# erkinov-wtf/dct

Hardware: AMD Instinct MI355X
Metric: 8x8 macroblocks/sec (DCT+quant); % HBM roofline (higher is better)
Workload: dtype fp32

## Files before the change

### dct_amd/__init__.py

```python
from __future__ import annotations

import ctypes as C
import os

HERE = os.path.dirname(os.path.abspath(__file__))
LIB_PATH = os.path.join(HERE, "libdct_amd.so")

KINDS = {"uniform": 0, "smooth": 1, "const": 2, "extreme": 3}


class DctqError(RuntimeError):
    pass


class _Plane(C.Structure):
    _fields_ = [("pixels", C.c_void_p), ("stride", C.c_longlong), ("frame_stride", C.c_longlong),
                ("width", C.c_int), ("height", C.c_int), ("nframes", C.c_int)]


_lib = None
_diag = None
DIAG_PATH = os.path.join(HERE, "libdct_amd_diag.so")


def _bind(L: C.CDLL, diagnostic: bool) -> C.CDLL:
    vp, i, ll = C.c_void_p, C.c_int, C.c_longlong
    sig = {
        "dctq_plan_create": ([i, i, C.POINTER(vp)], i),
        "dctq_plan_destroy": ([vp], None),
        "dctq_plan_set_fallback_counter": ([vp, vp], i),
        "dctq_forward_quant": ([vp, C.POINTER(_Plane), vp, vp, vp], i),
        "dctq_forward_quant_planes": ([vp, C.POINTER(_Plane), i, vp, vp, vp], i),
        "dctq_round_trip_planes": ([vp, C.POINTER(_Plane), i, vp, vp, vp, vp], i),
        "dctq_encode_workspace_bytes": ([ll], C.c_size_t),
        "dctq_encode_planes": ([vp, C.POINTER(_Plane), i, vp, vp, vp, ll, vp, vp], i),
        "dctq_encode_planes16": ([vp, C.POINTER(_Plane), i, vp, vp, vp, ll, vp, vp], i),
        "dctq_abi_version": ([], i),
        "dctq_forward_float": ([vp, C.POINTER(_Plane), vp, vp], i),
        "dctq_inverse": ([vp, vp, vp, ll, vp, vp], i),
        "dctq_decode_planes": ([vp, vp, vp, C.POINTER(_Plane), i, vp], i),
        "dctq_synth": ([C.c_uint64, i, C.POINTER(_Plane), vp], i),
        "dctq_error_string": ([i], C.c_char_p),
        "dctq_synchronize": ([vp], i),
        "dctq_rle_workspace_bytes": ([ll], C.c_size_t),
        "dctq_rle_count": ([vp, ll, vp, vp, vp], i),
        "dctq_rle_emit": ([vp, ll, vp, vp, vp], i),
        "dctq_rle_decode": ([vp, vp, ll, vp, vp], i),
        "dctq_rle_decode16": ([vp, vp, ll, vp, vp], i),
        "dctq_plan_symbol_bytes": ([vp], i),
        "dctq_huffman_bits": ([vp, ll, vp, vp], i),
        "dctq_huffman_bits_planes": ([vp, C.POINTER(_Plane), i, vp, vp], i),
        "dctq_stream_release": ([vp], i),
    }
    if diagnostic:
        sig.update({
            "dctq_diag_plan_set_variant": ([vp, i], i),
            "dctq_diag_forward_quant_planes": ([vp, C.POINTER(_Plane), i, vp, vp, vp], i),
            "dctq_diag_forward_float": ([vp, C.POINTER(_Plane), vp, vp], i),
            "dctq_diag_inverse": ([vp, vp, vp, ll, vp, vp], i),
            "dctq_diag_plan_set_num_cus": ([vp, i], i),
            "dctq_diag_plan_set_inverse": ([vp, i], i),
            "dctq_debug_inverse_bound": ([i, i, C.POINTER(i)], C.c_double),
            "dctq_debug_symbol_bytes": ([i, i], i),
            "dctq_diag_legacy_lanes": ([C.POINTER(i), C.POINTER(i)], i),
            "dctq_diag_movement_planes": ([vp, C.POINTER(_Plane), i, vp, vp], i),
            "dctq_diag_movement_v2_planes": ([vp, C.POINTER(_Plane), i, vp, vp], i),
            "dctq_diag_movement_grid_planes": ([vp, C.POINTER(_Plane), i, vp, i, vp], i),
            "dctq_diag_rt_movement_planes": ([vp, C.POINTER(_Plane), i, vp, vp, vp], i),
            "dctq_diag_stream": ([i, vp, vp, ll, vp], i),
            "dctq_diag_stream_release": ([vp], i),
            "dctq_debug_tables": ([i, i, vp, vp, vp, vp], i),
            "dctq_debug_fastdiv": ([C.c_uint32, C.c_uint32], i),
            "dctq_debug_dc_table": ([i, vp], i),
            "dctq_debug_forward_kernel": ([i, i, ll, i], i),
            "dctq_diag_stream_stash_bytes": ([vp], ll),
        })
    for name, (args, res) in sig.items():
        fn = getattr(L, name)
        fn.argtypes = args
        fn.restype = res
    return L


def lib() -> C.CDLL:
    global _lib
    if _lib is None:
        if not os.path.exists(LIB_PATH):
            raise DctqError(f"{LIB_PATH} is missing: run `python -m dct_amd.build` (hipcc, gfx950)")
        _lib = _bind(C.CDLL(LIB_PATH), False)
    return _lib


def diag() -> C.CDLL:
    global _diag
    if _diag is None:
        if not os.path.exists(DIAG_PATH):
            raise DctqError(f"{DIAG_PATH} is missing: run `python -m dct_amd.build` (hipcc, gfx950)")
        _diag = _bind(C.CDLL(DIAG_PATH), True)
    return _diag


def _check(rc: int, L: C.CDLL = None) -> None:
    if rc != 0:
        raise DctqError(f"dctq error {rc}: {(L or lib()).dctq_error_string(rc).decode()}")


def _need(t, numel: int, dtype, what: str, device=None):
    import torch
    if not isinstance(t, torch.Tensor) or not t.is_cuda:
        raise DctqError(f"{what} must be a tensor on a HIP device")
    if t.dtype != dtype:
        raise DctqError(f"{what} must be {dtype}, got {t.dtype}")
    if not t.is_contiguous():
        raise DctqError(f"{what} must be contiguous")
    if t.numel() < numel:
        raise DctqError(f"{what} holds {t.numel()} elements, {numel} needed")
    if device is not None and t.device != device:
        raise DctqError(f"{what} is on {t.device}, the input is on {device}")
    return t


def _stream_ptr(stream=None):
# ... 329 lines not shown
```

### dct_amd/build.py

```python
from __future__ import annotations

import os
import re
import subprocess
import sys

HERE = os.path.dirname(os.path.abspath(__file__))
ROOT = os.path.dirname(HERE)
CSRC = os.path.join(HERE, "csrc")
LIB = os.path.join(HERE, "libdct_amd.so")
DIAG_LIB = os.path.join(HERE, "libdct_amd_diag.so")
DIAG_SOURCES = ["diag.hip", "fdct8_diag.hip"]
SOURCES = ["api.hip", "legacy.hip", "fdct8.hip", "fdct8_aux.hip", "f64_pair.hip", "rle.hip", "roundtrip.hip", "encode.hip", "huffman.hip", "decode.hip"]
HEADERS = ["dctq_internal.h", "plan.h", "dctq_diag.h", "fdct8_bound.h", "idct8_bound.h", "host_tables.h", "aan_f64.h", "fdct8_core.h", "pair_core.h", "inverse_core.h", "scan_core.h", "zigzag.h"]
ARCH = "gfx950"


INFO = os.path.join(HERE, "build_info.json")


def _sha256(path: str) -> str:
    import hashlib
    with open(path, "rb") as f:
        return hashlib.sha256(f.read()).hexdigest()


def _inputs() -> dict:
    deps = [os.path.join(CSRC, f) for f in SOURCES + DIAG_SOURCES + HEADERS] + [os.path.abspath(__file__)]
    deps += [os.path.join(ROOT, "include", f) for f in sorted(os.listdir(os.path.join(ROOT, "include")))]
    return {os.path.relpath(d, ROOT): _sha256(d) for d in deps}


def build_info() -> dict:
    import json
    try:
        with open(INFO) as f:
            return json.load(f)
    except (OSError, ValueError):
        return {}


def _stale() -> bool:
    if not os.path.exists(LIB) or not os.path.exists(DIAG_LIB):
        return True
    info = build_info()
    return (info.get("inputs") != _inputs() or info.get("lib_sha256") != _sha256(LIB)
            or info.get("diag_sha256") != _sha256(DIAG_LIB) or info.get("flags") != _portable_flags())


def _portable_flags() -> list:
    return [f.replace(ROOT, "$ROOT") for f in _flags()]


def _flags():
    return ["hipcc", f"--offload-arch={ARCH}", "-O3", "-std=c++17", "-fPIC", "-ffp-contract=off",
            "-fno-slp-vectorize", "-Wall", "-Wno-unused-command-line-argument",
            "-I" + os.path.join(ROOT, "include"), "-I" + CSRC]


def declared_functions(headers) -> list:
    names = set()
    for h in headers:
        src = re.sub(r"/\*.*?\*/", "", open(h).read(), flags=re.S)
        for m in re.finditer(r"^[A-Za-z_][\w \*]*?\b([a-z_][a-z0-9_]*)\s*\(", src, flags=re.M):
            if m.group(1) not in ("if", "while", "for", "return", "sizeof", "defined"):
                names.add(m.group(1))
    return sorted(names)
# ... 60 lines not shown
```

### dct_amd/csrc/api.hip

```cpp
#include <dlfcn.h>
#include <math.h>
#include <stdio.h>
#include <stdlib.h>
#include <string.h>

#include <atomic>
#include <functional>
#include <map>
#include <mutex>
#include <string>
#include <thread>
#include <utility>
#include <vector>

#include "dct_amd.h"
#include "dctq_diag.h"
#include "dctq_internal.h"
#include "fdct8_bound.h"
#include "host_tables.h"
#include "idct8_bound.h"
#include "plan.h"

namespace {
thread_local std::string g_err;
// ... 419 lines not shown
                               symbols ? (unsigned long long)symbols_capacity : 0ull, workspace, (hipStream_t)stream,
                               plan->num_cus),
           "encode launch");
    return DCTQ_OK;
}

int dctq_encode_planes(const dctq_plan *plan, const dctq_plane *planes, int nplanes, int16_t *const *coef,
                       uint32_t *offsets, uint32_t *symbols, long long symbols_capacity, void *workspace,
                       void *stream) {
    DCTQ_LAUNCH(stream, 2);
    return encode_planes(plan, planes, nplanes, coef, offsets, symbols, symbols_capacity, workspace, stream, 4);
}

int dctq_encode_planes16(const dctq_plan *plan, const dctq_plane *planes, int nplanes, int16_t *const *coef,
                         uint32_t *offsets, uint16_t *symbols, long long symbols_capacity, void *workspace,
                         void *stream) {
    DCTQ_LAUNCH(stream, 13);
    return encode_planes(plan, planes, nplanes, coef, offsets, symbols, symbols_capacity, workspace, stream, 2);
}

int dctq_forward_quant(const dctq_plan *plan, const dctq_plane *src, int16_t *coef, int32_t *var_num, void *stream) {
    if (!src) return fail(DCTQ_EINVAL, "plane is NULL");
    return dctq_forward_quant_planes(plan, src, 1, &coef, var_num ? &var_num : nullptr, stream);
}

int dctq_forward_float(const dctq_plan *plan, const dctq_plane *src, float *coef, void *stream) {
    DCTQ_LAUNCH(stream, 3);
    if (int rc = dctq::check_plan(plan)) return rc;
    if (!coef) return fail(DCTQ_EINVAL, "coef is NULL");
    if (((uintptr_t)coef) % 16) return fail(DCTQ_EINVAL, "coef must be 16-byte aligned");
    dctq::PlaneArgs a;
    int rc = dctq::plane_args(src, &a);
    if (rc) return rc;
    HIPCHK(dctq::launch_fdct8_float_pair(a, plan->dev, coef, (hipStream_t)stream, plan->num_cus),
           "fdct8_float_pair launch");
    return DCTQ_OK;
}

int dctq_inverse(const dctq_plan *plan, const int16_t *coef, const int32_t *var_num, long long nblocks, float *recon,
                 void *stream) {
    DCTQ_LAUNCH(stream, 4);
    if (int rc = dctq::check_plan(plan)) return rc;
    if (!coef || !recon) return fail(DCTQ_EINVAL, "coef/recon is NULL");
    if (plan->adaptive && !var_num) return fail(DCTQ_EINVAL, "adaptive inverse needs var_num");
    if (nblocks < 0 || nblocks >= (1ll << 40)) return fail(DCTQ_EINVAL, "bad nblocks");
    if (((uintptr_t)coef) % 16 || ((uintptr_t)recon) % 16) return fail(DCTQ_EINVAL, "coef/recon must be 16-byte aligned");
    if (nblocks == 0) return DCTQ_OK;
    HIPCHK(dctq::launch_idct8_pair(plan->dev, plan->adaptive, coef, var_num, nblocks, recon, (hipStream_t)stream,
                                   plan->num_cus),
           "idct8_pair launch");
    return DCTQ_OK;
}

int dctq_decode_planes(const dctq_plan *plan, const int16_t *const *coef, const int32_t *const *var_num,
                       const dctq_plane *dst, int nplanes, void *stream) {
    DCTQ_LAUNCH(stream, 14);
    if (int rc = dctq::check_plan(plan)) return rc;
    if (!coef || !dst) return fail(DCTQ_EINVAL, "coef/dst is NULL");
    if (nplanes < 1 || nplanes > dctq::kMaxPlanes) return fail(DCTQ_EINVAL, "nplanes must be in [1, 4]");
    if (plan->adaptive && !var_num) return fail(DCTQ_EINVAL, "adaptive decode needs var_num");
    dctq::DecodeSet ds = {};
    ds.n = nplanes;
    uint32_t first = 0;
    for (int k = 0; k < nplanes; ++k) {
        if (int rc = dctq::plane_args(&dst[k], &ds.pl[k])) return rc;
        if (!coef[k]) return fail(DCTQ_EINVAL, "coef[k] is NULL");
        if (((uintptr_t)coef[k]) % 16) return fail(DCTQ_EINVAL, "coef must be 16-byte aligned");
        if (plan->adaptive && !var_num[k]) return fail(DCTQ_EINVAL, "adaptive decode needs every var_num[k]");
        ds.coef[k] = coef[k];
        ds.var[k] = plan->adaptive ? var_num[k] : nullptr;
        ds.first[k] = first;
        first += (uint32_t)((ds.pl[k].nblk + 31) / 32);
    }
    for (int k = nplanes; k <= dctq::kMaxPlanes; ++k) ds.first[k] = first;
    HIPCHK(dctq::launch_decode(ds, plan->dev, plan->adaptive, plan->inv_f32 != 0, (hipStream_t)stream, plan->num_cus),
           "decode launch");
    return DCTQ_OK;
}

int dctq_synth(uint64_t seed, int kind, const dctq_plane *dst, void *stream) {
    DCTQ_LAUNCH(stream, 5);
    if (!dst || !dst->pixels) return fail(DCTQ_EINVAL, "dst is NULL");
    if (dst->width <= 0 || dst->height <= 0 || dst->width % 4 || dst->stride < dst->width || dst->stride % 4 ||
        dst->nframes < 1 || ((uintptr_t)dst->pixels) % 4)
        return fail(DCTQ_EINVAL, "bad synth plane geometry");
    HIPCHK(dctq::launch_synth(seed, kind, (uint8_t *)dst->pixels, dst->stride, dst->frame_stride, dst->width,
                              dst->height, dst->nframes, (hipStream_t)stream),
           "synth launch");
    return DCTQ_OK;
}

static int device_cus() {
    int dev = 0, n = 0;
    if (hipGetDevice(&dev) != hipSuccess) return 256;
    if (hipDeviceGetAttribute(&n, hipDeviceAttributeMultiprocessorCount, dev) != hipSuccess || n < 1) return 256;
    return n;
}

static int rle_args(const void *a, const void *b, long long nblocks) {
    if (!a || !b) return fail(DCTQ_EINVAL, "NULL pointer");
    if (nblocks < 1 || nblocks >= (1ll << 26)) return fail(DCTQ_EINVAL, "nblocks must be in [1, 2^26)");
    return DCTQ_OK;
}

size_t dctq_rle_workspace_bytes(long long nblocks) { return dctq::rle_workspace_bytes(nblocks < 1 ? 1 : nblocks); }

int dctq_rle_count(const int16_t *coef, long long nblocks, uint32_t *offsets, void *workspace, void *stream) {
    DCTQ_LAUNCH(stream, 6);
    if (int rc = rle_args(coef, offsets, nblocks)) return rc;
    if (!workspace) return fail(DCTQ_EINVAL, "workspace is NULL");
    HIPCHK(dctq::launch_rle_count(coef, nblocks, offsets, workspace, (hipStream_t)stream, device_cus()),
           "rle_count launch");
    return DCTQ_OK;
}

int dctq_rle_emit(const int16_t *coef, long long nblocks, const uint32_t *offsets, uint32_t *symbols, void *stream) {
    DCTQ_LAUNCH(stream, 7);
    if (int rc = rle_args(coef, offsets, nblocks)) return rc;
    if (!symbols) return fail(DCTQ_EINVAL, "symbols is NULL");
    HIPCHK(dctq::launch_rle_emit(coef, nblocks, offsets, symbols, 4, ~0ull, (hipStream_t)stream, device_cus()),
           "rle_emit launch");
    return DCTQ_OK;
}

int dctq_rle_decode(const uint32_t *symbols, const uint32_t *offsets, long long nblocks, int16_t *coef,
                    void *stream) {
    DCTQ_LAUNCH(stream, 8);
// ... 98 lines not shown
```

### dct_amd/csrc/dctq_diag.h

```cpp
#ifndef DCTQ_DIAG_H
#define DCTQ_DIAG_H

#include "dct_amd.h"

#ifdef __cplusplus
extern "C" {
#endif

int dctq_diag_plan_set_variant(dctq_plan *plan, int variant);
int dctq_diag_forward_quant_planes(const dctq_plan *plan, const dctq_plane *planes, int nplanes, int16_t *const *coef,
                                   int32_t *const *var_num, void *stream);
int dctq_diag_forward_float(const dctq_plan *plan, const dctq_plane *src, float *coef, void *stream);
int dctq_diag_inverse(const dctq_plan *plan, const int16_t *coef, const int32_t *var_num, long long nblocks,
                      float *recon, void *stream);

int dctq_diag_plan_set_inverse(dctq_plan *plan, int mode);

int dctq_diag_plan_set_num_cus(dctq_plan *plan, int num_cus);

int dctq_diag_movement_planes(const dctq_plan *plan, const dctq_plane *planes, int nplanes, int16_t *const *coef,
                              void *stream);
int dctq_diag_movement_grid_planes(const dctq_plan *plan, const dctq_plane *planes, int nplanes, int16_t *const *coef,
                                   int grid_mult, void *stream);
int dctq_diag_movement_v2_planes(const dctq_plan *plan, const dctq_plane *planes, int nplanes, int16_t *const *coef,
                                 void *stream);

int dctq_diag_rt_movement_planes(const dctq_plan *plan, const dctq_plane *planes, int nplanes, int16_t *const *coef,
                                 float *const *recon, void *stream);

int dctq_diag_stream(int kind, const void *src, void *dst, long long blocks, void *stream);

int dctq_diag_stream_release(void *stream);
long long dctq_diag_stream_stash_bytes(void *stream);

int dctq_debug_forward_kernel(int quality, int adaptive, long long batches, int num_cus);
int dctq_debug_tables(int quality, int adaptive, float *w, float *thr, double *dct, double *quant);
int dctq_debug_dc_table(int quality, int16_t *out);
int dctq_debug_fastdiv(uint32_t d, uint32_t n);
double dctq_debug_inverse_bound(int quality, int adaptive, int *admitted);
int dctq_debug_symbol_bytes(int quality, int adaptive);
int dctq_diag_legacy_lanes(int *made, int *pooled);

#ifdef __cplusplus
}
#endif
#endif
```

### dct_amd/csrc/decode.hip

```cpp
#include "inverse_core.h"

namespace dctq {

constexpr int kDecodeGridMult = 64;

__device__ __forceinline__ const int16_t *coef_in(const DecodeSet &ds, int k) {
    const int16_t *c = ds.coef[0];
#pragma unroll
    for (int i = 1; i < kMaxPlanes; ++i) c = k == i ? ds.coef[i] : c;
    return c;
}
__device__ __forceinline__ const int32_t *var_in(const DecodeSet &ds, int k) {
    const int32_t *v = ds.var[0];
#pragma unroll
    for (int i = 1; i < kMaxPlanes; ++i) v = k == i ? ds.var[i] : v;
    return v;
}
__device__ __forceinline__ uint32_t first_batch(const DecodeSet &ds, int k) {
    uint32_t f = 0u;
#pragma unroll
    for (int i = 1; i < kMaxPlanes; ++i) f = k == i ? ds.first[i] : f;
    return f;
}
__device__ __forceinline__ int plane_of_batch(const DecodeSet &ds, uint32_t g) {
    int k = 0;
#pragma unroll
    for (int i = 1; i < kMaxPlanes; ++i) k += (i < ds.n && g >= ds.first[i]) ? 1 : 0;
    return k;
}

template <bool ADAPTIVE>
__device__ __forceinline__ void prefetch_coefs(const DecodeSet &ds, uint32_t g, int h, int j, uint4 (&rows)[4],
                                               int32_t &vn) {
    const int k = plane_of_batch(ds, g);
    const uint32_t n = (g - first_batch(ds, k)) * 32u + (uint32_t)j;
    const uint32_t m = n < (uint32_t)ds.pl[k].nblk ? n : 0u;
    const u4p *src = reinterpret_cast<const u4p *>(coef_in(ds, k) + (size_t)m * 64) + 4 * h;
#pragma unroll
    for (int r = 0; r < 4; ++r) {
        const u4p t = __builtin_nontemporal_load(src + r);
        rows[r] = make_uint4(t.x, t.y, t.z, t.w);
    }
    if (ADAPTIVE) vn = __builtin_nontemporal_load(var_in(ds, k) + m);
}

__device__ __forceinline__ uint32_t pack_u8x4(float a, float b, float c, float d) {
    uint32_t w = 0u;
    w = __builtin_amdgcn_cvt_pk_u8_f32(__builtin_rintf(__builtin_amdgcn_fmed3f(a, 0.0f, 255.0f)), 0u, w);
    w = __builtin_amdgcn_cvt_pk_u8_f32(__builtin_rintf(__builtin_amdgcn_fmed3f(b, 0.0f, 255.0f)), 1u, w);
    w = __builtin_amdgcn_cvt_pk_u8_f32(__builtin_rintf(__builtin_amdgcn_fmed3f(c, 0.0f, 255.0f)), 2u, w);
    w = __builtin_amdgcn_cvt_pk_u8_f32(__builtin_rintf(__builtin_amdgcn_fmed3f(d, 0.0f, 255.0f)), 3u, w);
    return w;
}

template <bool ADAPTIVE, bool INV32>
__global__ __launch_bounds__(kThreadsP, 4) void decode8(DecodeSet ds, const DevTables *__restrict__ dev) {
    const int lane = threadIdx.x & 63, wv = __builtin_amdgcn_readfirstlane(threadIdx.x >> 6);
    const int h = lane >> 5, j = lane & 31;
    const uint32_t nbatch = ds.first[kMaxPlanes];
    const uint32_t step = gridDim.x * kWavesP;
    uint32_t g = blockIdx.x * kWavesP + wv;
    uint4 nxt[4];
    int32_t nvn = 0;
    prefetch_coefs<ADAPTIVE>(ds, g, h, j, nxt, nvn);
    for (; g < nbatch; g += step) {
        const int k = plane_of_batch(ds, g);
        const PlaneArgs &p = ds.pl[k];
        const uint32_t n = (g - first_batch(ds, k)) * 32u + (uint32_t)j;
        const bool valid = n < (uint32_t)p.nblk;
        uint4 cur[4];
#pragma unroll
        for (int r = 0; r < 4; ++r) cur[r] = nxt[r];
        const int32_t vn = nvn;
        prefetch_coefs<ADAPTIVE>(ds, g + step, h, j, nxt, nvn);

        u2p pix[4];
        const auto pack = [&pix](int r, int c, const float (&o)[4]) { pix[r][c >> 2] = pack_u8x4(o[0], o[1], o[2], o[3]); };
        if constexpr (INV32) inverse_half_f32_rows(dev, cur, h, pack);
        else inverse_half_rows<ADAPTIVE>(dev, cur, vn, h, pack);

        const uint32_t m = valid ? n : 0u;
        const uint32_t f = fdiv(m, p.div_frame);
        const uint32_t rem = m - f * (uint32_t)p.nblk_frame;
        const uint32_t by = fdiv(rem, p.div_bw);
        const uint32_t bx = rem - by * (uint32_t)p.bw;
        uint8_t *base = const_cast<uint8_t *>(p.src);
        if (p.span) {
            const __amdgpu_buffer_rsrc_t rs = __builtin_amdgcn_make_buffer_rsrc(base, (short)0, (int)p.span, 0x00020000);
            const uint32_t st = (uint32_t)p.stride;
            const uint32_t off = f * (uint32_t)p.frame_stride + (by * 8u + 4u * (uint32_t)h) * st + bx * 8u;
            if (valid) {
#pragma unroll
                for (int r = 0; r < 4; ++r) __builtin_amdgcn_raw_buffer_store_b64(pix[r], rs, off + r * st, 0, kNtAux);
            }
        } else if (valid) {
            uint8_t *px = base + (long long)f * p.frame_stride + (long long)(by * 8u + 4u * (uint32_t)h) * p.stride +
                          (long long)bx * 8;
#pragma unroll
            for (int r = 0; r < 4; ++r) __builtin_nontemporal_store(pix[r], reinterpret_cast<u2p *>(px + r * p.stride));
        }
    }
}

template <bool A, bool F32>
static hipError_t launch_dec(const DecodeSet &ds, const DevTables *dev, hipStream_t stream, int num_cus) {
    static const int per_cu = resident_per_cu(decode8<A, F32>, kThreadsP);
    const uint32_t nbatch = ds.first[kMaxPlanes];
    const uint32_t want = (nbatch + kWavesP - 1) / kWavesP;
    const uint32_t cap = (uint32_t)(num_cus * per_cu * kDecodeGridMult);
    hipLaunchKernelGGL((decode8<A, F32>), dim3(want < cap ? want : cap), dim3(kThreadsP), 0, stream, ds, dev);
    return hipGetLastError();
}

hipError_t launch_decode(const DecodeSet &ds, const DevTables *dev, int adaptive, bool inv_f32, hipStream_t stream,
                         int num_cus) {
    if (adaptive) return launch_dec<true, false>(ds, dev, stream, num_cus);
    if (inv_f32) return launch_dec<false, true>(ds, dev, stream, num_cus);
    return launch_dec<false, false>(ds, dev, stream, num_cus);
}

}
```

### dct_amd/csrc/diag.hip

```cpp
#include <string.h>

#include "dctq_diag.h"
#include "fdct8_bound.h"
#include "host_tables.h"
#include "plan.h"

namespace dctq {
namespace {

typedef unsigned int u4v __attribute__((ext_vector_type(4)));
typedef unsigned int u2v2 __attribute__((ext_vector_type(2)));

template <int AUX>
__global__ __launch_bounds__(256) void stream12(const u4v *__restrict__ src, char *__restrict__ dst, uint32_t nb) {
    const int lane = threadIdx.x & 63;
    for (uint32_t b = blockIdx.x * 4 + (threadIdx.x >> 6); b < nb; b += gridDim.x * 4) {
        u4v v[4];
#pragma unroll
        for (int k = 0; k < 4; ++k) v[k] = __builtin_nontemporal_load(src + (size_t)b * 256 + k * 64 + lane);
        const __amdgpu_buffer_rsrc_t rc = __builtin_amdgcn_make_buffer_rsrc(dst + (size_t)b * 8192, 0, 8192, 0x00020000);
#pragma unroll
        for (int k = 0; k < 4; ++k) {
            __builtin_amdgcn_raw_buffer_store_b128(v[k], rc, lane * 16, k * 1024, AUX);
            __builtin_amdgcn_raw_buffer_store_b128(v[k] ^ u4v{1, 0, 0, 0}, rc, lane * 16, (k + 4) * 1024, AUX);
        }
    }
}

__global__ __launch_bounds__(256) void stream124(const u4v *__restrict__ src, char *__restrict__ dst, uint32_t nb) {
    const int lane = threadIdx.x & 63;
    for (uint32_t b = blockIdx.x * 4 + (threadIdx.x >> 6); b < nb; b += gridDim.x * 4) {
        u4v v[4];
#pragma unroll
        for (int k = 0; k < 4; ++k) v[k] = __builtin_nontemporal_load(src + (size_t)b * 256 + k * 64 + lane);
        const __amdgpu_buffer_rsrc_t rc =
            __builtin_amdgcn_make_buffer_rsrc(dst + (size_t)b * 24576, 0, 24576, 0x00020000);
#pragma unroll
        for (int k = 0; k < 4; ++k)
#pragma unroll
            for (int m = 0; m < 6; ++m)
                __builtin_amdgcn_raw_buffer_store_b128(v[k] ^ u4v{(unsigned)m, 0, 0, 0}, rc, lane * 16,
                                                       (k * 6 + m) * 1024, 2);
    }
}

template <bool GROUPS>
__global__ __launch_bounds__(256) void stream124_split(const u4v *__restrict__ src, char *__restrict__ dst,
                                                       uint32_t nb) {
    const int lane = threadIdx.x & 63;
    for (uint32_t b = blockIdx.x * 4 + (threadIdx.x >> 6); b < nb; b += gridDim.x * 4) {
        u4v v[4];
#pragma unroll
        for (int k = 0; k < 4; ++k) v[k] = __builtin_nontemporal_load(src + (size_t)b * 256 + k * 64 + lane);
        const __amdgpu_buffer_rsrc_t ra = __builtin_amdgcn_make_buffer_rsrc(dst + (size_t)b * 8192, 0, 8192, 0x00020000);
        const __amdgpu_buffer_rsrc_t rb =
// ... 90 lines not shown
            for (int k = 0; k < 4; ++k)
#pragma unroll
                for (int m = 0; m < 2; ++m)
                    __builtin_amdgcn_raw_buffer_store_b128(v[k] ^ u4v{(unsigned)(2 + 2 * h + m), 0, 0, 0}, rb,
                                                           lane * 16, (h * 8 + k * 2 + m) * 1024, 2);
        }
    }
}

__global__ __launch_bounds__(256) void stream12_plane(const uint8_t *__restrict__ src, char *__restrict__ dst,
                                                      uint32_t nb) {
    constexpr uint32_t kW = 3840, kBpr = kW / 8;
    const int lane = threadIdx.x & 63;
    const __amdgpu_buffer_rsrc_t rs =
        __builtin_amdgcn_make_buffer_rsrc(const_cast<uint8_t *>(src), (short)0, (int)(nb * 4096u), 0x00020000);
    const uint32_t nfull = nb * 64u / kBpr * kBpr;
    for (uint32_t b = blockIdx.x * 4 + (threadIdx.x >> 6); b < nb; b += gridDim.x * 4) {
        const uint32_t n = (b * 64u + (uint32_t)lane) % nfull;
        const uint32_t off = (n / kBpr) * 8u * kW + (n % kBpr) * 8u;
        u2v2 r[8];
#pragma unroll
        for (int y = 0; y < 8; ++y) r[y] = __builtin_amdgcn_raw_buffer_load_b64(rs, off + y * kW, 0, 2);
        const __amdgpu_buffer_rsrc_t rc = __builtin_amdgcn_make_buffer_rsrc(dst + (size_t)b * 8192, 0, 8192, 0x00020000);
#pragma unroll
        for (int k = 0; k < 4; ++k) {
            const u4v v = u4v{r[2 * k].x, r[2 * k].y, r[2 * k + 1].x, r[2 * k + 1].y};
            __builtin_amdgcn_raw_buffer_store_b128(v, rc, lane * 16, k * 1024, 2);
            __builtin_amdgcn_raw_buffer_store_b128(v ^ u4v{1, 0, 0, 0}, rc, lane * 16, (k + 4) * 1024, 2);
        }
    }
}

__global__ __launch_bounds__(256) void stream_read(const u4v *__restrict__ src, u4v *__restrict__ sink, size_t n16) {
    const size_t base = (size_t)blockIdx.x * 1024 + threadIdx.x;
    u4v acc = {0, 0, 0, 0};
#pragma unroll
    for (int u = 0; u < 4; ++u)
        if (base + u * 256 < n16) acc ^= __builtin_nontemporal_load(src + base + u * 256);
    if (acc.x == 0x12345678u && acc.y == 0x9abcdef0u && acc.z == 0x0fedcba9u) sink[0] = acc;
}

template <bool NT>
__global__ __launch_bounds__(256) void stream_write(u4v *__restrict__ dst, size_t n16) {
    const size_t base = (size_t)blockIdx.x * 1024 + threadIdx.x;
#pragma unroll
    for (int u = 0; u < 4; ++u)
        if (base + u * 256 < n16) {
            const u4v v = u4v{(unsigned)base, (unsigned)u, 7u, 9u};
            if (NT) __builtin_nontemporal_store(v, dst + base + u * 256);
            else dst[base + u * 256] = v;
        }
}

int device_cus() {
    int dev = 0, n = 0;
    if (hipGetDevice(&dev) != hipSuccess) return 256;
    if (hipDeviceGetAttribute(&n, hipDeviceAttributeMultiprocessorCount, dev) != hipSuccess || n < 1) return 256;
    return n;
}

}
}

extern "C" {

int dctq_diag_plan_set_variant(dctq_plan *plan, int variant) {
    DCTQ_ENTRY;
    if (!plan) return dctq::fail(DCTQ_EINVAL, "plan is NULL");
    if (variant < 1 || variant > 4) return dctq::fail(DCTQ_EINVAL, "variant must be 1..4");
    plan->variant = variant;
    return DCTQ_OK;
}

int dctq_diag_plan_set_inverse(dctq_plan *plan, int mode) {
    DCTQ_ENTRY;
    if (!plan) return dctq::fail(DCTQ_EINVAL, "plan is NULL");
    if (mode != 0 && mode != 1) return dctq::fail(DCTQ_EINVAL, "mode must be 0 (fp64) or 1 (the plan's own choice)");
    plan->inv_f32 = mode == 1 && !plan->adaptive && plan->inv_bound <= kInvTolDiag;
    return DCTQ_OK;
}

double dctq_debug_inverse_bound(int quality, int adaptive, int *admitted) {
    dctq::DevTables t;
    dctq_host::dct_matrix(8, t.dct);
    dctq_host::quant_matrix(8, dctq_host::clamp_quality(quality), t.quant);
    for (int c = 0; c < 64; ++c) {
        t.dequant[c] = 1.0 / t.quant[c];
        t.s2[c] = kAanScale[c >> 3] * kAanScale[c & 7];
    }
    const double b = dctq::inverse_f32_bound(t);
    if (admitted) *admitted = !adaptive && b <= kInvTolDiag;
    return b;
}

int dctq_diag_legacy_lanes(int *made, int *pooled) {
    if (!made || !pooled) return dctq::fail(DCTQ_EINVAL, "NULL pointer");
    dctq::legacy_lane_counts(made, pooled);
    return DCTQ_OK;
}

int dctq_debug_symbol_bytes(int quality, int adaptive) {
    (void)adaptive;
    dctq::DevTables t;
    dctq_host::dct_matrix(8, t.dct);
    dctq_host::quant_matrix(8, dctq_host::clamp_quality(quality), t.quant);
    return dctq::max_abs_quantized(t) <= 511 ? 2 : 4;
// ... 1 lines not shown

int dctq_diag_plan_set_num_cus(dctq_plan *plan, int num_cus) {
    DCTQ_ENTRY;
    if (!plan) return dctq::fail(DCTQ_EINVAL, "plan is NULL");
    if (num_cus < 1 || num_cus > 4096) return dctq::fail(DCTQ_EINVAL, "num_cus must be 1..4096");
    plan->num_cus = num_cus;
    return DCTQ_OK;
}

int dctq_diag_movement_planes(const dctq_plan *plan, const dctq_plane *planes, int nplanes, int16_t *const *coef,
                              void *stream) {
    DCTQ_ENTRY;
    if (int rc = dctq::check_plan(plan)) return rc;
    dctq::PlaneSet ps;
    if (int rc = dctq::plane_set(planes, nplanes, coef, nullptr, &ps)) return rc;
    HIPCHK(dctq::launch_fdct8_movement(ps, plan->dev, (hipStream_t)stream, plan->num_cus, 3), "fdct8_movement launch");
    return DCTQ_OK;
}

int dctq_diag_movement_grid_planes(const dctq_plan *plan, const dctq_plane *planes, int nplanes, int16_t *const *coef,
                                   int grid_mult, void *stream) {
    DCTQ_ENTRY;
    if (int rc = dctq::check_plan(plan)) return rc;
    if (grid_mult < 1 || grid_mult > 64) return dctq::fail(DCTQ_EINVAL, "grid_mult must be 1..64");
    dctq::PlaneSet ps;
    if (int rc = dctq::plane_set(planes, nplanes, coef, nullptr, &ps)) return rc;
    HIPCHK(dctq::launch_fdct8_movement(ps, plan->dev, (hipStream_t)stream, plan->num_cus, 3, grid_mult),
           "fdct8_movement launch");
    return DCTQ_OK;
}

int dctq_diag_movement_v2_planes(const dctq_plan *plan, const dctq_plane *planes, int nplanes, int16_t *const *coef,
                                 void *stream) {
    DCTQ_ENTRY;
    if (int rc = dctq::check_plan(plan)) return rc;
    dctq::PlaneSet ps;
    if (int rc = dctq::plane_set(planes, nplanes, coef, nullptr, &ps)) return rc;
    HIPCHK(dctq::launch_fdct8_movement(ps, plan->dev, (hipStream_t)stream, plan->num_cus, 2), "fdct8_movement_v2 launch");
    return DCTQ_OK;
}

int dctq_diag_rt_movement_planes(const dctq_plan *plan, const dctq_plane *planes, int nplanes, int16_t *const *coef,
                                 float *const *recon, void *stream) {
    DCTQ_ENTRY;
    if (int rc = dctq::check_plan(plan)) return rc;
    if (!recon) return dctq::fail(DCTQ_EINVAL, "recon is NULL");
    dctq::RoundTripSet rt = {};
    if (int rc = dctq::plane_set(planes, nplanes, coef, nullptr, &rt.ps)) return rc;
    for (int k = 0; k < nplanes; ++k) {
        if (!recon[k] || ((uintptr_t)recon[k]) % 16) return dctq::fail(DCTQ_EINVAL, "recon[k] NULL or misaligned");
        rt.recon[k] = recon[k];
    }
    HIPCHK(dctq::launch_roundtrip_movement(rt, (hipStream_t)stream, plan->num_cus), "roundtrip_movement launch");
    return DCTQ_OK;
}

int dctq_diag_stream(int kind, const void *src, void *dst, long long blocks, void *stream) {
    DCTQ_ENTRY;
    using namespace dctq;
    if (!src || !dst || ((uintptr_t)src) % 16 || ((uintptr_t)dst) % 16) return fail(DCTQ_EINVAL, "src/dst NULL or misaligned");
    if (blocks < 64 || blocks % 64 || blocks >= (1ll << 31)) return fail(DCTQ_EINVAL, "blocks must be a multiple of 64 in [64, 2^31)");
    const uint32_t nb = (uint32_t)(blocks / 64);
    const hipStream_t s = (hipStream_t)stream;
    const int grid = device_cus() * 4;
    switch (kind) {
    case 0: hipLaunchKernelGGL(stream12<2>, dim3(grid), dim3(256), 0, s, (const u4v *)src, (char *)dst, nb); break;
    case 1: hipLaunchKernelGGL(stream12<0>, dim3(grid), dim3(256), 0, s, (const u4v *)src, (char *)dst, nb); break;
    case 2: {
        const size_t n16 = (size_t)blocks * 4;
        hipLaunchKernelGGL(stream_read, dim3((unsigned)((n16 + 1023) / 1024)), dim3(256), 0, s, (const u4v *)src,
                           (u4v *)dst, n16);
        break;
    }
    case 3:
    case 4: {
        const size_t n16 = (size_t)blocks * 8;
        if (kind == 3)
            hipLaunchKernelGGL(stream_write<false>, dim3((unsigned)((n16 + 1023) / 1024)), dim3(256), 0, s, (u4v *)dst, n16);
        else
            hipLaunchKernelGGL(stream_write<true>, dim3((unsigned)((n16 + 1023) / 1024)), dim3(256), 0, s, (u4v *)dst, n16);
        break;
    }
    case 5: hipLaunchKernelGGL(stream124, dim3(grid), dim3(256), 0, s, (const u4v *)src, (char *)dst, nb); break;
    case 6:
    case 7: {
        const unsigned want = (nb + 3) / 4, g = (unsigned)grid * (kind == 6 ? 16u : 32u);
        hipLaunchKernelGGL(stream12<2>, dim3(g < want ? g : want), dim3(256), 0, s, (const u4v *)src, (char *)dst, nb);
        break;
    }
    case 8: hipLaunchKernelGGL(stream124_split<false>, dim3(grid), dim3(256), 0, s, (const u4v *)src, (char *)dst, nb); break;
    case 9: hipLaunchKernelGGL(stream124_split<true>, dim3(grid), dim3(256), 0, s, (const u4v *)src, (char *)dst, nb); break;
    case 10: hipLaunchKernelGGL(stream124_rows<0>, dim3(grid), dim3(256), 0, s, (const uint8_t *)src, (char *)dst, nb); break;
    case 11: hipLaunchKernelGGL(stream124_rows<3840>, dim3(grid), dim3(256), 0, s, (const uint8_t *)src, (char *)dst, nb); break;
    case 12: hipLaunchKernelGGL((stream124_rows<3840, 1>), dim3(grid), dim3(256), 0, s, (const uint8_t *)src, (char *)dst, nb); break;
    case 13: hipLaunchKernelGGL((stream124_rows<3840, 2>), dim3(grid), dim3(256), 0, s, (const uint8_t *)src, (char *)dst, nb); break;
    case 14: {
        const unsigned want = (nb + 3) / 4, g = (unsigned)grid * 32u;
        hipLaunchKernelGGL(stream12_plane, dim3(g < want ? g : want), dim3(256), 0, s, (const uint8_t *)src, (char *)dst, nb);
        break;
    }
    case 15: hipLaunchKernelGGL(stream124_rows16, dim3(grid), dim3(256), 0, s, (const uint8_t *)src, (char *)dst, nb); break;
    case 16:
    case 17: {
        const unsigned want = (nb + 3) / 4, g = (unsigned)grid * 32u;
        if (kind == 16)
            hipLaunchKernelGGL(stream124_split<true>, dim3(g < want ? g : want), dim3(256), 0, s, (const u4v *)src,
// ... 48 lines not shown
```

### dct_amd/csrc/plan.h

```cpp
#pragma once
#include <hip/hip_runtime.h>

#include "dct_amd.h"
#include "dctq_internal.h"

struct dctq_plan {
    int quality, adaptive, device, num_cus;
    int variant;
    dctq::FastTables fast;
    dctq::DevTables host;
    dctq::DevTables *dev;
    unsigned long long *fallbacks;
    int inv_f32;
    double inv_bound;
    int symbol_bytes;
};

namespace dctq {
int fail(int code, const char *what, hipError_t e = hipSuccess);
int check_plan(const dctq_plan *plan);
int plane_args(const dctq_plane *s, PlaneArgs *a);
int plane_inputs(const dctq_plane *planes, int nplanes, PlaneSet *ps);
int plane_set(const dctq_plane *planes, int nplanes, int16_t *const *coef, int32_t *const *var_num, PlaneSet *ps);
void fill_fast_tables(const double *q, int adaptive, FastTables *t);
void dc_const_table(const double *d, const double *q, int16_t *tab);
double inverse_f32_bound(const DevTables &t);
int max_abs_quantized(const DevTables &t);
}
constexpr double kInvTolDiag = 5e-5;
namespace dctq {
}

#define HIPCHK(call, what)                                               \
    do {                                                                 \
        hipError_t e_ = (call);                                          \
        if (e_ != hipSuccess) return ::dctq::fail(DCTQ_EHIP, what, e_); \
    } while (0)
```

Measured before the change: 31.64 billion.

## Stage decode coefficients and pixels through LDS in 64-block tiles

The decode kernel now loads 64 blocks of coefficients per wave as contiguous 128-bit buffer loads, stages them in LDS, runs the inverse transform from LDS, stages the packed pixels back into LDS, and stores full 8-row blocks per lane. This replaces per-lane strided half-block loads and half-block stores, aiming for coalesced reads and wider per-lane writes. The grid multiplier drops from 64 to 16, and diagnostic movement kernels plus a stream21 kernel are added to measure the data path alone. The cost is LDS traffic, extra wave syncs and higher shared-memory use per block. The measured metric is forward DCT+quant, which this decode path may not affect.

```diff
diff --git a/dct_amd/__init__.py b/dct_amd/__init__.py
--- a/dct_amd/__init__.py
+++ b/dct_amd/__init__.py
@@ -68,6 +68,8 @@
             "dctq_diag_movement_grid_planes": ([vp, C.POINTER(_Plane), i, vp, i, vp], i),
             "dctq_diag_rt_movement_planes": ([vp, C.POINTER(_Plane), i, vp, vp, vp], i),
             "dctq_diag_stream": ([i, vp, vp, ll, vp], i),
+            "dctq_diag_decode_movement_planes": ([vp, vp, C.POINTER(_Plane), i, i, i, vp], i),
+            "dctq_diag_stream21": ([vp, vp, ll, i, vp], i),
             "dctq_diag_stream_release": ([vp], i),
             "dctq_debug_tables": ([i, i, vp, vp, vp, vp], i),
             "dctq_debug_fastdiv": ([C.c_uint32, C.c_uint32], i),
diff --git a/dct_amd/build.py b/dct_amd/build.py
--- a/dct_amd/build.py
+++ b/dct_amd/build.py
@@ -12,7 +12,7 @@
 DIAG_LIB = os.path.join(HERE, "libdct_amd_diag.so")
 DIAG_SOURCES = ["diag.hip", "fdct8_diag.hip"]
 SOURCES = ["api.hip", "legacy.hip", "fdct8.hip", "fdct8_aux.hip", "f64_pair.hip", "rle.hip", "roundtrip.hip", "encode.hip", "huffman.hip", "decode.hip"]
-HEADERS = ["dctq_internal.h", "plan.h", "dctq_diag.h", "fdct8_bound.h", "idct8_bound.h", "host_tables.h", "aan_f64.h", "fdct8_core.h", "pair_core.h", "inverse_core.h", "scan_core.h", "zigzag.h"]
+HEADERS = ["dctq_internal.h", "plan.h", "dctq_diag.h", "fdct8_bound.h", "idct8_bound.h", "host_tables.h", "aan_f64.h", "fdct8_core.h", "pair_core.h", "inverse_core.h", "decode_core.h", "scan_core.h", "zigzag.h"]
 ARCH = "gfx950"
 
 
diff --git a/dct_amd/csrc/api.hip b/dct_amd/csrc/api.hip
--- a/dct_amd/csrc/api.hip
+++ b/dct_amd/csrc/api.hip
@@ -495,13 +495,13 @@
     return DCTQ_OK;
 }
 
-int dctq_decode_planes(const dctq_plan *plan, const int16_t *const *coef, const int32_t *const *var_num,
-                       const dctq_plane *dst, int nplanes, void *stream) {
-    DCTQ_LAUNCH(stream, 14);
-    if (int rc = dctq::check_plan(plan)) return rc;
+}
+
+int dctq::decode_set(const int16_t *const *coef, const int32_t *const *var_num, bool adaptive, const dctq_plane *dst,
+                     int nplanes, int tile, dctq::DecodeSet *out) {
     if (!coef || !dst) return fail(DCTQ_EINVAL, "coef/dst is NULL");
     if (nplanes < 1 || nplanes > dctq::kMaxPlanes) return fail(DCTQ_EINVAL, "nplanes must be in [1, 4]");
-    if (plan->adaptive && !var_num) return fail(DCTQ_EINVAL, "adaptive decode needs var_num");
+    if (adaptive && !var_num) return fail(DCTQ_EINVAL, "adaptive decode needs var_num");
     dctq::DecodeSet ds = {};
     ds.n = nplanes;
     uint32_t first = 0;
@@ -509,13 +509,25 @@
         if (int rc = dctq::plane_args(&dst[k], &ds.pl[k])) return rc;
         if (!coef[k]) return fail(DCTQ_EINVAL, "coef[k] is NULL");
         if (((uintptr_t)coef[k]) % 16) return fail(DCTQ_EINVAL, "coef must be 16-byte aligned");
-        if (plan->adaptive && !var_num[k]) return fail(DCTQ_EINVAL, "adaptive decode needs every var_num[k]");
+        if (adaptive && !var_num[k]) return fail(DCTQ_EINVAL, "adaptive decode needs every var_num[k]");
         ds.coef[k] = coef[k];
-        ds.var[k] = plan->adaptive ? var_num[k] : nullptr;
+        ds.var[k] = adaptive ? var_num[k] : nullptr;
         ds.first[k] = first;
-        first += (uint32_t)((ds.pl[k].nblk + 31) / 32);
+        first += (uint32_t)((ds.pl[k].nblk + tile - 1) / tile);
     }
     for (int k = nplanes; k <= dctq::kMaxPlanes; ++k) ds.first[k] = first;
+    *out = ds;
+    return DCTQ_OK;
+}
+
+extern "C" {
+
+int dctq_decode_planes(const dctq_plan *plan, const int16_t *const *coef, const int32_t *const *var_num,
+                       const dctq_plane *dst, int nplanes, void *stream) {
+    DCTQ_LAUNCH(stream, 14);
+    if (int rc = dctq::check_plan(plan)) return rc;
+    dctq::DecodeSet ds;
+    if (int rc = dctq::decode_set(coef, var_num, plan->adaptive != 0, dst, nplanes, 64, &ds)) return rc;
     HIPCHK(dctq::launch_decode(ds, plan->dev, plan->adaptive, plan->inv_f32 != 0, (hipStream_t)stream, plan->num_cus),
            "decode launch");
     return DCTQ_OK;
diff --git a/dct_amd/csrc/dctq_diag.h b/dct_amd/csrc/dctq_diag.h
--- a/dct_amd/csrc/dctq_diag.h
+++ b/dct_amd/csrc/dctq_diag.h
@@ -28,6 +28,10 @@
 int dctq_diag_rt_movement_planes(const dctq_plan *plan, const dctq_plane *planes, int nplanes, int16_t *const *coef,
                                  float *const *recon, void *stream);
 
+int dctq_diag_decode_movement_planes(const dctq_plan *plan, const int16_t *const *coef, const dctq_plane *dst,
+                                     int nplanes, int shape, int grid_mult, void *stream);
+int dctq_diag_stream21(const void *src, void *dst, long long blocks, int grid_mult, void *stream);
+
 int dctq_diag_stream(int kind, const void *src, void *dst, long long blocks, void *stream);
 
 int dctq_diag_stream_release(void *stream);
diff --git a/dct_amd/csrc/decode.hip b/dct_amd/csrc/decode.hip
--- a/dct_amd/csrc/decode.hip
+++ b/dct_amd/csrc/decode.hip
@@ -1,48 +1,6 @@
-#include "inverse_core.h"
+#include "decode_core.h"
 
 namespace dctq {
-
-constexpr int kDecodeGridMult = 64;
-
-__device__ __forceinline__ const int16_t *coef_in(const DecodeSet &ds, int k) {
-    const int16_t *c = ds.coef[0];
-#pragma unroll
-    for (int i = 1; i < kMaxPlanes; ++i) c = k == i ? ds.coef[i] : c;
-    return c;
-}
-__device__ __forceinline__ const int32_t *var_in(const DecodeSet &ds, int k) {
-    const int32_t *v = ds.var[0];
-#pragma unroll
-    for (int i = 1; i < kMaxPlanes; ++i) v = k == i ? ds.var[i] : v;
-    return v;
-}
-__device__ __forceinline__ uint32_t first_batch(const DecodeSet &ds, int k) {
-    uint32_t f = 0u;
-#pragma unroll
-    for (int i = 1; i < kMaxPlanes; ++i) f = k == i ? ds.first[i] : f;
-    return f;
-}
-__device__ __forceinline__ int plane_of_batch(const DecodeSet &ds, uint32_t g) {
-    int k = 0;
-#pragma unroll
-    for (int i = 1; i < kMaxPlanes; ++i) k += (i < ds.n && g >= ds.first[i]) ? 1 : 0;
-    return k;
-}
-
-template <bool ADAPTIVE>
-__device__ __forceinline__ void prefetch_coefs(const DecodeSet &ds, uint32_t g, int h, int j, uint4 (&rows)[4],
-                                               int32_t &vn) {
-    const int k = plane_of_batch(ds, g);
-    const uint32_t n = (g - first_batch(ds, k)) * 32u + (uint32_t)j;
-    const uint32_t m = n < (uint32_t)ds.pl[k].nblk ? n : 0u;
-    const u4p *src = reinterpret_cast<const u4p *>(coef_in(ds, k) + (size_t)m * 64) + 4 * h;
-#pragma unroll
-    for (int r = 0; r < 4; ++r) {
-        const u4p t = __builtin_nontemporal_load(src + r);
-        rows[r] = make_uint4(t.x, t.y, t.z, t.w);
-    }
-    if (ADAPTIVE) vn = __builtin_nontemporal_load(var_in(ds, k) + m);
-}
 
 __device__ __forceinline__ uint32_t pack_u8x4(float a, float b, float c, float d) {
     uint32_t w = 0u;
@@ -54,59 +12,56 @@
 }
 
 template <bool ADAPTIVE, bool INV32>
+__device__ __forceinline__ void decode_half(const DevTables *__restrict__ dev, char *wstage, int b, int h, int32_t vn) {
+    uint4 q[4];
+    staged_half(wstage, b, h, q);
+    wave_sync();
+    u2p pix[4];
+    const auto pack = [&pix](int r, int c, const float (&o)[4]) { pix[r][c >> 2] = pack_u8x4(o[0], o[1], o[2], o[3]); };
+    if constexpr (INV32) inverse_half_f32_rows(dev, q, h, pack);
+    else inverse_half_rows<ADAPTIVE>(dev, q, vn, h, pack);
+    stage_pixels(wstage, b, h, pix);
+}
+
+template <bool ADAPTIVE, bool INV32>
 __global__ __launch_bounds__(kThreadsP, 4) void decode8(DecodeSet ds, const DevTables *__restrict__ dev) {
+    __shared__ uint4 stage[kWavesP * kDecodeStage / 16];
     const int lane = threadIdx.x & 63, wv = __builtin_amdgcn_readfirstlane(threadIdx.x >> 6);
-    const int h = lane >> 5, j = lane & 31;
-    const uint32_t nbatch = ds.first[kMaxPlanes];
+    const uint32_t ntile = ds.first[kMaxPlanes];
     const uint32_t step = gridDim.x * kWavesP;
     uint32_t g = blockIdx.x * kWavesP + wv;
-    uint4 nxt[4];
+    char *wstage = reinterpret_cast<char *>(stage) + wv * kDecodeStage;
+    u4p nxt[8] = {};
     int32_t nvn = 0;
-    prefetch_coefs<ADAPTIVE>(ds, g, h, j, nxt, nvn);
-    for (; g < nbatch; g += step) {
-        const int k = plane_of_batch(ds, g);
+    prefetch_tile<ADAPTIVE>(ds, g, lane, nxt, nvn);
+    for (; g < ntile; g += step) {
+        const int k = plane_of_tile(ds, g);
         const PlaneArgs &p = ds.pl[k];
-        const uint32_t n = (g - first_batch(ds, k)) * 32u + (uint32_t)j;
-        const bool valid = n < (uint32_t)p.nblk;
-        uint4 cur[4];
-#pragma unroll
-        for (int r = 0; r < 4; ++r) cur[r] = nxt[r];
+        const uint32_t t = g - first_tile(ds, k);
+
+        retire_stores();
+        stage_tile(wstage, lane, nxt);
         const int32_t vn = nvn;
-        prefetch_coefs<ADAPTIVE>(ds, g + step, h, j, nxt, nvn);
+        prefetch_tile<ADAPTIVE>(ds, g + step, lane, nxt, nvn);
+        wave_sync();
 
-        u2p pix[4];
-        const auto pack = [&pix](int r, int c, const float (&o)[4]) { pix[r][c >> 2] = pack_u8x4(o[0], o[1], o[2], o[3]); };
-        if constexpr (INV32) inverse_half_f32_rows(dev, cur, h, pack);
-        else inverse_half_rows<ADAPTIVE>(dev, cur, vn, h, pack);
+        int ol = lane;
+        asm volatile("" : "+v"(ol));
+        const int h = ol >> 5, j = ol & 31;
+        const auto vv = __builtin_amdgcn_permlane32_swap((uint32_t)vn, (uint32_t)vn, false, false);
+        decode_half<ADAPTIVE, INV32>(dev, wstage, j, h, (int32_t)vv[0]);
+        decode_half<ADAPTIVE, INV32>(dev, wstage, 32 + j, h, (int32_t)vv[1]);
+        wave_sync();
 
-        const uint32_t m = valid ? n : 0u;
-        const uint32_t f = fdiv(m, p.div_frame);
-        const uint32_t rem = m - f * (uint32_t)p.nblk_frame;
-        const uint32_t by = fdiv(rem, p.div_bw);
-        const uint32_t bx = rem - by * (uint32_t)p.bw;
-        uint8_t *base = const_cast<uint8_t *>(p.src);
-        if (p.span) {
-            const __amdgpu_buffer_rsrc_t rs = __builtin_amdgcn_make_buffer_rsrc(base, (short)0, (int)p.span, 0x00020000);
-            const uint32_t st = (uint32_t)p.stride;
-            const uint32_t off = f * (uint32_t)p.frame_stride + (by * 8u + 4u * (uint32_t)h) * st + bx * 8u;
-            if (valid) {
-#pragma unroll
-                for (int r = 0; r < 4; ++r) __builtin_amdgcn_raw_buffer_store_b64(pix[r], rs, off + r * st, 0, kNtAux);
-            }
-        } else if (valid) {
-            uint8_t *px = base + (long long)f * p.frame_stride + (long long)(by * 8u + 4u * (uint32_t)h) * p.stride +
-                          (long long)bx * 8;
-#pragma unroll
-            for (int r = 0; r < 4; ++r) __builtin_nontemporal_store(pix[r], reinterpret_cast<u2p *>(px + r * p.stride));
-        }
+        store_tile_rows(p, wstage, t, lane);
     }
 }
 
 template <bool A, bool F32>
 static hipError_t launch_dec(const DecodeSet &ds, const DevTables *dev, hipStream_t stream, int num_cus) {
     static const int per_cu = resident_per_cu(decode8<A, F32>, kThreadsP);
-    const uint32_t nbatch = ds.first[kMaxPlanes];
-    const uint32_t want = (nbatch + kWavesP - 1) / kWavesP;
+    const uint32_t ntile = ds.first[kMaxPlanes];
+    const uint32_t want = (ntile + kWavesP - 1) / kWavesP;
     const uint32_t cap = (uint32_t)(num_cus * per_cu * kDecodeGridMult);
     hipLaunchKernelGGL((decode8<A, F32>), dim3(want < cap ? want : cap), dim3(kThreadsP), 0, stream, ds, dev);
     return hipGetLastError();
diff --git a/dct_amd/csrc/decode_core.h b/dct_amd/csrc/decode_core.h
--- /dev/null
+++ b/dct_amd/csrc/decode_core.h
@@ -0,0 +1,114 @@
+#pragma once
+#include "inverse_core.h"
+
+namespace dctq {
+
+constexpr int kDecodeGridMult = 16;
+constexpr int kPixPitch = 72;
+constexpr int kDecodeStage = 64 * kPitch2;
+static_assert(kPixPitch <= kPitch2, "half A's pixels (blocks 0-31) stay below block 32's coefficients, read after them");
+
+__device__ __forceinline__ const int16_t *coef_in(const DecodeSet &ds, int k) {
+    const int16_t *c = ds.coef[0];
+#pragma unroll
+    for (int i = 1; i < kMaxPlanes; ++i) c = k == i ? ds.coef[i] : c;
+    return c;
+}
+__device__ __forceinline__ const int32_t *var_in(const DecodeSet &ds, int k) {
+    const int32_t *v = ds.var[0];
+#pragma unroll
+    for (int i = 1; i < kMaxPlanes; ++i) v = k == i ? ds.var[i] : v;
+    return v;
+}
+__device__ __forceinline__ uint32_t first_tile(const DecodeSet &ds, int k) {
+    uint32_t f = 0u;
+#pragma unroll
+    for (int i = 1; i < kMaxPlanes; ++i) f = k == i ? ds.first[i] : f;
+    return f;
+}
+__device__ __forceinline__ int plane_of_tile(const DecodeSet &ds, uint32_t g) {
+    int k = 0;
+#pragma unroll
+    for (int i = 1; i < kMaxPlanes; ++i) k += (i < ds.n && g >= ds.first[i]) ? 1 : 0;
+    return k;
+}
+
+template <bool ADAPTIVE>
+__device__ __forceinline__ void prefetch_tile(const DecodeSet &ds, uint32_t g, int lane, u4p (&nxt)[8], int32_t &vn) {
+    if (g >= ds.first[kMaxPlanes]) return;
+    const int k = plane_of_tile(ds, g);
+    const uint32_t t = g - first_tile(ds, k);
+    const uint32_t left = (uint32_t)ds.pl[k].nblk - t * 64u;
+    const uint32_t nb = left < 64u ? left : 64u;
+    const __amdgpu_buffer_rsrc_t rs = __builtin_amdgcn_make_buffer_rsrc(
+        const_cast<int16_t *>(coef_in(ds, k)) + (size_t)t * 4096, (short)0, (int)(nb * 128u), 0x00020000);
+#pragma unroll
+    for (int c = 0; c < 8; ++c) nxt[c] = __builtin_amdgcn_raw_buffer_load_b128(rs, lane * 16 + c * 1024, 0, 2 );
+    if (ADAPTIVE) {
+        const __amdgpu_buffer_rsrc_t rv = __builtin_amdgcn_make_buffer_rsrc(
+            const_cast<int32_t *>(var_in(ds, k)) + (size_t)t * 64, (short)0, (int)(nb * 4u), 0x00020000);
+        vn = (int32_t)__builtin_amdgcn_raw_buffer_load_b32(rv, lane * 4, 0, 2);
+    }
+}
+
+__device__ __forceinline__ void stage_tile(char *wstage, int lane, const u4p (&v)[8]) {
+#pragma unroll
+    for (int c = 0; c < 8; ++c) {
+        const int m = c * 64 + lane;
+        uint2 *d = reinterpret_cast<uint2 *>(wstage + (m >> 3) * kPitch2 + (m & 7) * 16);
+        d[0] = make_uint2(v[c].x, v[c].y);
+        d[1] = make_uint2(v[c].z, v[c].w);
+    }
+}
+
+__device__ __forceinline__ void staged_half(const char *wstage, int b, int h, uint4 (&q)[4]) {
+    const uint2 *s = reinterpret_cast<const uint2 *>(wstage) + b * (kPitch2 / 8) + h * 8;
+#pragma unroll
+    for (int r = 0; r < 4; ++r) {
+        const uint2 lo = s[2 * r], hi = s[2 * r + 1];
+        q[r] = make_uint4(lo.x, lo.y, hi.x, hi.y);
+    }
+}
+
+__device__ __forceinline__ void stage_pixels(char *wstage, int b, int h, const u2p (&pix)[4]) {
+    u2p *d = reinterpret_cast<u2p *>(wstage + b * kPixPitch + h * 32);
+#pragma unroll
+    for (int r = 0; r < 4; ++r) d[r] = pix[r];
+}
+
+__device__ __forceinline__ void block_pos(const PlaneArgs &p, uint32_t n, uint32_t &f, uint32_t &by, uint32_t &bx) {
+    f = fdiv(n, p.div_frame);
+    const uint32_t rem = n - f * (uint32_t)p.nblk_frame;
+    by = fdiv(rem, p.div_bw);
+    bx = rem - by * (uint32_t)p.bw;
+}
+
+__device__ __forceinline__ void store_tile_rows(const PlaneArgs &p, const char *wstage, uint32_t t, int lane) {
+    uint8_t *base = const_cast<uint8_t *>(p.src);
+    const uint32_t n = t * 64u + (uint32_t)lane;
+    const bool valid = n < (uint32_t)p.nblk;
+    uint32_t f, by, bx;
+    block_pos(p, valid ? n : 0u, f, by, bx);
+    const uint2 *s = reinterpret_cast<const uint2 *>(wstage + lane * kPixPitch);
+    u2p v[8];
+#pragma unroll
+    for (int r = 0; r < 8; ++r) {
+        const uint2 a = s[r];
+        v[r] = u2p{a.x, a.y};
+    }
+    if (p.span) {
+        const __amdgpu_buffer_rsrc_t rs = __builtin_amdgcn_make_buffer_rsrc(base, (short)0, (int)p.span, 0x00020000);
+        const uint32_t st = (uint32_t)p.stride;
+        const uint32_t off = f * (uint32_t)p.frame_stride + by * 8u * st + bx * 8u;
+        if (valid) {
+#pragma unroll
+            for (int r = 0; r < 8; ++r) __builtin_amdgcn_raw_buffer_store_b64(v[r], rs, off + r * st, 0, kNtAux);
+        }
+    } else if (valid) {
+        uint8_t *px = base + (long long)f * p.frame_stride + (long long)(by * 8u) * p.stride + (long long)bx * 8;
+#pragma unroll
+        for (int r = 0; r < 8; ++r) __builtin_nontemporal_store(v[r], reinterpret_cast<u2p *>(px + r * p.stride));
+    }
+}
+
+}
diff --git a/dct_amd/csrc/diag.hip b/dct_amd/csrc/diag.hip
--- a/dct_amd/csrc/diag.hip
+++ b/dct_amd/csrc/diag.hip
@@ -1,6 +1,7 @@
 #include <string.h>
 
 #include "dctq_diag.h"
+#include "decode_core.h"
 #include "fdct8_bound.h"
 #include "host_tables.h"
 #include "plan.h"
@@ -197,6 +198,93 @@
         }
 }
 
+__global__ __launch_bounds__(kThreadsP, 4) void dec_movement_tiles(DecodeSet ds) {
+    __shared__ uint4 stage[kWavesP * kDecodeStage / 16];
+    const int lane = threadIdx.x & 63, wv = __builtin_amdgcn_readfirstlane(threadIdx.x >> 6);
+    const uint32_t ntile = ds.first[kMaxPlanes];
+    const uint32_t step = gridDim.x * kWavesP;
+    uint32_t g = blockIdx.x * kWavesP + wv;
+    char *wstage = reinterpret_cast<char *>(stage) + wv * kDecodeStage;
+    u4p nxt[8] = {};
+    int32_t nvn = 0;
+    prefetch_tile<false>(ds, g, lane, nxt, nvn);
+    for (; g < ntile; g += step) {
+        const int k = plane_of_tile(ds, g);
+        const uint32_t t = g - first_tile(ds, k);
+        retire_stores();
+        stage_tile(wstage, lane, nxt);
+        prefetch_tile<false>(ds, g + step, lane, nxt, nvn);
+        wave_sync();
+        const int h = lane >> 5, j = lane & 31;
+#pragma unroll
+        for (int half = 0; half < 2; ++half) {
+            uint4 q[4];
+            staged_half(wstage, 32 * half + j, h, q);
+            wave_sync();
+            u2p pix[4];
+#pragma unroll
+            for (int r = 0; r < 4; ++r) pix[r] = u2p{q[r].x ^ q[r].z, q[r].y ^ q[r].w};
+            stage_pixels(wstage, 32 * half + j, h, pix);
+        }
+        wave_sync();
+        store_tile_rows(ds.pl[k], wstage, t, lane);
+    }
+}
+
+__global__ __launch_bounds__(kThreadsP, 4) void dec_movement_rows(DecodeSet ds) {
+    const int lane = threadIdx.x & 63, wv = __builtin_amdgcn_readfirstlane(threadIdx.x >> 6);
+    const int h = lane >> 5, j = lane & 31;
+    const uint32_t nbatch = ds.first[kMaxPlanes];
+    const uint32_t step = gridDim.x * kWavesP;
+    const auto load = [&](uint32_t g, u4p (&rows)[4]) {
+        const int k = plane_of_tile(ds, g);
+        const uint32_t n = (g - first_tile(ds, k)) * 32u + (uint32_t)j;
+        const uint32_t m = n < (uint32_t)ds.pl[k].nblk ? n : 0u;
+        const u4p *src = reinterpret_cast<const u4p *>(coef_in(ds, k) + (size_t)m * 64) + 4 * h;
+#pragma unroll
+        for (int r = 0; r < 4; ++r) rows[r] = __builtin_nontemporal_load(src + r);
+    };
+    uint32_t g = blockIdx.x * kWavesP + wv;
+    u4p nxt[4];
+    load(g, nxt);
+    for (; g < nbatch; g += step) {
+        const int k = plane_of_tile(ds, g);
+        const PlaneArgs &p = ds.pl[k];
+        const uint32_t n = (g - first_tile(ds, k)) * 32u + (uint32_t)j;
+        const bool valid = n < (uint32_t)p.nblk;
+        u2p pix[4];
+#pragma unroll
+        for (int r = 0; r < 4; ++r) pix[r] = u2p{nxt[r].x ^ nxt[r].z, nxt[r].y ^ nxt[r].w};
+        load(g + step, nxt);
+        uint32_t f, by, bx;
+        block_pos(p, valid ? n : 0u, f, by, bx);
+        const __amdgpu_buffer_rsrc_t rs =
+            __builtin_amdgcn_make_buffer_rsrc(const_cast<uint8_t *>(p.src), (short)0, (int)p.span, 0x00020000);
+        const uint32_t st = (uint32_t)p.stride;
+        const uint32_t off = f * (uint32_t)p.frame_stride + (by * 8u + 4u * (uint32_t)h) * st + bx * 8u;
+        if (valid) {
+#pragma unroll
+            for (int r = 0; r < 4; ++r) __builtin_amdgcn_raw_buffer_store_b64(pix[r], rs, off + r * st, 0, kNtAux);
+        }
+    }
+}
+
+__global__ __launch_bounds__(256) void stream21(const char *__restrict__ src, char *__restrict__ dst, uint32_t blocks) {
+    const int lane = threadIdx.x & 63;
+    const uint32_t nt = (blocks + 63u) / 64u;
+    for (uint32_t b = blockIdx.x * 4 + (threadIdx.x >> 6); b < nt; b += gridDim.x * 4) {
+        const uint32_t left = blocks - b * 64u, nb = left < 64u ? left : 64u;
+        const __amdgpu_buffer_rsrc_t rl =
+            __builtin_amdgcn_make_buffer_rsrc(const_cast<char *>(src) + (size_t)b * 8192, 0, (int)(nb * 128u), 0x00020000);
+        const __amdgpu_buffer_rsrc_t rc = __builtin_amdgcn_make_buffer_rsrc(dst + (size_t)b * 4096, 0, (int)(nb * 64u), 0x00020000);
+        u4v v[8];
+#pragma unroll
+        for (int k = 0; k < 8; ++k) v[k] = __builtin_amdgcn_raw_buffer_load_b128(rl, lane * 16 + k * 1024, 0, 2);
+#pragma unroll
+        for (int k = 0; k < 4; ++k) __builtin_amdgcn_raw_buffer_store_b128(v[2 * k] ^ v[2 * k + 1], rc, lane * 16 + k * 1024, 0, 2);
+    }
+}
+
 int device_cus() {
     int dev = 0, n = 0;
     if (hipGetDevice(&dev) != hipSuccess) return 256;
@@ -304,6 +392,46 @@
         rt.recon[k] = recon[k];
     }
     HIPCHK(dctq::launch_roundtrip_movement(rt, (hipStream_t)stream, plan->num_cus), "roundtrip_movement launch");
+    return DCTQ_OK;
+}
+
+int dctq_diag_decode_movement_planes(const dctq_plan *plan, const int16_t *const *coef, const dctq_plane *dst,
+                                     int nplanes, int shape, int grid_mult, void *stream) {
+    DCTQ_ENTRY;
+    using namespace dctq;
+    if (int rc = check_plan(plan)) return rc;
+    if (shape != 0 && shape != 1) return fail(DCTQ_EINVAL, "shape must be 0 (32-block row batches) or 1 (64-block tiles)");
+    if (grid_mult < 0 || grid_mult > 64) return fail(DCTQ_EINVAL, "grid_mult must be 0..64");
+    DecodeSet ds;
+    if (int rc = decode_set(coef, nullptr, false, dst, nplanes, shape ? 64 : 32, &ds)) return rc;
+    for (int k = 0; k < nplanes; ++k)
+        if (!ds.pl[k].span) return fail(DCTQ_EINVAL, "planes of 4 GiB or more are not measured");
+    const uint32_t n = ds.first[kMaxPlanes], want = (n + kWavesP - 1) / kWavesP;
+    const int mult = grid_mult ? grid_mult : shape ? kDecodeGridMult : 64;
+    if (shape) {
+        static const int per_cu = resident_per_cu(dec_movement_tiles, kThreadsP);
+        const uint32_t cap = (uint32_t)(plan->num_cus * per_cu * mult);
+        hipLaunchKernelGGL(dec_movement_tiles, dim3(want < cap ? want : cap), dim3(kThreadsP), 0, (hipStream_t)stream, ds);
+    } else {
+        static const int per_cu = resident_per_cu(dec_movement_rows, kThreadsP);
+        const uint32_t cap = (uint32_t)(plan->num_cus * per_cu * mult);
+        hipLaunchKernelGGL(dec_movement_rows, dim3(want < cap ? want : cap), dim3(kThreadsP), 0, (hipStream_t)stream, ds);
+    }
+    HIPCHK(hipGetLastError(), "decode movement launch");
+    return DCTQ_OK;
+}
+
+int dctq_diag_stream21(const void *src, void *dst, long long blocks, int grid_mult, void *stream) {
+    DCTQ_ENTRY;
+    using namespace dctq;
+    if (!src || !dst || ((uintptr_t)src) % 16 || ((uintptr_t)dst) % 16) return fail(DCTQ_EINVAL, "src/dst NULL or misaligned");
+    if (blocks < 1 || blocks >= (1ll << 31)) return fail(DCTQ_EINVAL, "blocks must be in [1, 2^31)");
+    if (grid_mult < 1 || grid_mult > 64) return fail(DCTQ_EINVAL, "grid_mult must be 1..64");
+    const uint32_t nt = (uint32_t)((blocks + 63) / 64), want = (nt + 3) / 4;
+    const uint32_t cap = (uint32_t)device_cus() * 4u * (uint32_t)grid_mult;
+    hipLaunchKernelGGL(stream21, dim3(want < cap ? want : cap), dim3(256), 0, (hipStream_t)stream, (const char *)src,
+                       (char *)dst, (uint32_t)blocks);
+    HIPCHK(hipGetLastError(), "diag stream21 launch");
     return DCTQ_OK;
 }
 
diff --git a/dct_amd/csrc/plan.h b/dct_amd/csrc/plan.h
--- a/dct_amd/csrc/plan.h
+++ b/dct_amd/csrc/plan.h
@@ -22,6 +22,8 @@
 int plane_args(const dctq_plane *s, PlaneArgs *a);
 int plane_inputs(const dctq_plane *planes, int nplanes, PlaneSet *ps);
 int plane_set(const dctq_plane *planes, int nplanes, int16_t *const *coef, int32_t *const *var_num, PlaneSet *ps);
+int decode_set(const int16_t *const *coef, const int32_t *const *var_num, bool adaptive, const dctq_plane *dst,
+               int nplanes, int tile, DecodeSet *ds);
 void fill_fast_tables(const double *q, int adaptive, FastTables *t);
 void dc_const_table(const double *d, const double *q, int16_t *tab);
 double inverse_f32_bound(const DevTables &t);
```

Result: slower. 30.08 billion (-4.9%).
